# urbste/MultiCol-SLAM

Hardware: AMD Instinct MI355X
Metric: Mfeatures/s extract+match, 3-cam 754x480 multi-frame (higher is better)
Workload: dtype u8+i32 (images, Hamming) / f64 (omni model)

## Files before the change

multicol-slam_amd/csrc/mcs_blur.hip:

```cpp
#include "mcs_common.h"
#include <type_traits>

namespace mcs {

constexpr int kBlurRows = 32;
constexpr int kBlurAhead = 4;

struct BlurLevel { int waveBase, wavesX, rows, ncg; };
struct BlurPlan { int nlevels, totalWaves; BlurLevel lv[MCS_MAX_LEVELS]; };

__device__ __forceinline__ int reflect101(int p, int len) {
	p = p < 0 ? -p : p;
	return p >= len ? 2 * (len - 1) - p : p;
}

__global__ __launch_bounds__(256) void k_blur(ExtractBuffers b, BlurPlan plan, int nimg) {
	const PyrDesc& d = *b.desc;
	const int blk = (blockIdx.x & (kNumXCD - 1)) * (gridDim.x / kNumXCD) + (blockIdx.x / kNumXCD);
	const int wave = __builtin_amdgcn_readfirstlane(blk * 4 + (threadIdx.x >> 6));
	if (wave >= plan.totalWaves) return;
	int level = 0;
	while (level + 1 < plan.nlevels && wave >= plan.lv[level + 1].waveBase) ++level;
	const BlurLevel pl = plan.lv[level];
	const LevelInfo& L = d.lv[level];
	const int w = L.w, h = L.h, dstride = L.stride, pyrBytes = d.pyrBytes;
	const int wl = wave - pl.waveBase;
	const int rb = wl / pl.wavesX, wx = wl - rb * pl.wavesX;
	const int y0 = rb * pl.rows;
	const int nrows = min(pl.rows, h - y0);
	const int items = nimg * pl.ncg;
	const int item0 = wx * 64;
	const int itemRaw = item0 + (threadIdx.x & 63);
	const bool live = itemRaw < items;
	const int item = live ? itemRaw : items - 1;
	const int img = item / pl.ncg, cg = item - img * pl.ncg;
	const int img0 = item0 / pl.ncg;
	const int x = cg * 4;
	int sstride;
	const uint8_t* src = level_ptr(b, d, img0, level, &sstride);
	const size_t simg = level == 0 ? b.img0Pitch : (size_t)pyrBytes;
	uint8_t* dst = b.blur + (size_t)img0 * pyrBytes + L.off;
	const int A = min(max(x - 2, 0), w - 8);
	uint32_t selLo = 0, selHi = 0;
#pragma unroll
	for (int j = 0; j < 8; ++j) {
		const int p = reflect101(min(x - 2 + j, w + 1), w);
// ... 1 lines not shown
		if (j < 4) selLo |= s << (8 * j); else selHi |= s << (8 * (j - 4));
	}
	uint32_t voffS = (uint32_t)((size_t)(img - img0) * simg) + (uint32_t)A;
	uint32_t voffD = (uint32_t)((size_t)(img - img0) * (size_t)pyrBytes) + (uint32_t)x;
	auto loadRow = [&](int it) -> uint2 {
		const int r = reflect101(y0 - 2 + it, h);
		asm volatile("" : "+v"(voffS));
		uint2 v;
		__builtin_memcpy(&v, src + (size_t)((unsigned)r * (unsigned)sstride) + voffS, 8);
		return v;
	};
	const int total = nrows + 4;
	uint2 buf[5];
#pragma unroll
	for (int k = 0; k < kBlurAhead; ++k) buf[k] = loadRow(min(k, total - 1));
	uint32_t ring[5][4];
	uint32_t V[4] = {12u, 12u, 12u, 12u};
	auto body = [&](int it, auto kc, auto firstc, auto storec) {
		constexpr int k = decltype(kc)::value;
		buf[(k + kBlurAhead) % 5] = loadRow(min(it + kBlurAhead, total - 1));
		const uint2 raw = buf[k];
		const uint32_t W0 = __builtin_amdgcn_perm(raw.y, raw.x, selLo), W1 = __builtin_amdgcn_perm(raw.y, raw.x, selHi);
		uint32_t S[4];
		S[0] = __builtin_amdgcn_udot4(W0, 0x01010101u, W1 & 0xffu, false);
		S[1] = __builtin_amdgcn_udot4(W0, 0x01010100u, __builtin_amdgcn_udot4(W1, 0x00000101u, 0u, false), false);
		S[2] = __builtin_amdgcn_udot4(W0, 0x01010000u, __builtin_amdgcn_udot4(W1, 0x00010101u, 0u, false), false);
		S[3] = __builtin_amdgcn_udot4(W0, 0x01000000u, __builtin_amdgcn_udot4(W1, 0x01010101u, 0u, false), false);
#pragma unroll
		for (int c = 0; c < 4; ++c) {
			V[c] += S[c];
			if (!decltype(firstc)::value) V[c] -= ring[k][c];
			ring[k][c] = S[c];
		}
		if (decltype(storec)::value) {
			const uint32_t t0 = __umul24(V[0], 671104u), t1 = __umul24(V[1], 671104u), t2 = __umul24(V[2], 671104u), t3 = __umul24(V[3], 671104u);
			const uint32_t out = __builtin_amdgcn_perm(t1, t0, 0x0c0c0703u) | __builtin_amdgcn_perm(t3, t2, 0x07030c0cu);
			asm volatile("" : "+v"(voffD));
			*reinterpret_cast<uint32_t*>(dst + (size_t)((unsigned)(y0 + it - 4) * (unsigned)dstride) + voffD) = out;
		}
	};
	using T = std::true_type; using F = std::false_type;
	body(0, std::integral_constant<int, 0>(), T(), F()); body(1, std::integral_constant<int, 1>(), T(), F()); body(2, std::integral_constant<int, 2>(), T(), F());
	body(3, std::integral_constant<int, 3>(), T(), F()); body(4, std::integral_constant<int, 4>(), T(), T());
	int it0 = 5;
	for (; it0 + 5 <= total; it0 += 5) {
		body(it0, std::integral_constant<int, 0>(), F(), T()); body(it0 + 1, std::integral_constant<int, 1>(), F(), T()); body(it0 + 2, std::integral_constant<int, 2>(), F(), T());
		body(it0 + 3, std::integral_constant<int, 3>(), F(), T()); body(it0 + 4, std::integral_constant<int, 4>(), F(), T());
	}
	const int rem = total - it0;
	if (rem > 0) body(it0, std::integral_constant<int, 0>(), F(), T());
	if (rem > 1) body(it0 + 1, std::integral_constant<int, 1>(), F(), T());
	if (rem > 2) body(it0 + 2, std::integral_constant<int, 2>(), F(), T());
	if (rem > 3) body(it0 + 3, std::integral_constant<int, 3>(), F(), T());
}

void launch_blur(const ExtractBuffers& b, const PyrDesc& hd, int nimg, hipStream_t s) {
	BlurPlan plan;
	plan.nlevels = hd.nlevels;
	int waves = 0;
	for (int l = 0; l < hd.nlevels; ++l) {
		BlurLevel& p = plan.lv[l];
		const int w = hd.lv[l].w, h = hd.lv[l].h;
		p.ncg = (w + 3) / 4;
		const int nrb = (h + kBlurRows - 1) / kBlurRows;
		p.rows = (h + nrb - 1) / nrb;
		p.wavesX = (nimg * p.ncg + 63) / 64;
		p.waveBase = waves;
		waves += p.wavesX * ((h + p.rows - 1) / p.rows);
	}
	plan.totalWaves = waves;
	hipLaunchKernelGGL(k_blur, dim3(((waves + 3) / 4 + kNumXCD - 1) / kNumXCD * kNumXCD), dim3(256), 0, s, b, plan, nimg);
}

}
```

multicol-slam_amd/csrc/mcs_capi.hip:

```cpp
#include "mcs_extractor.h"
#include "mcs_plan.h"

#include <cstdio>
#include <cstdlib>

namespace mcs {
bool upload_describe_tables(const signed char* pattern);
const signed char kPattern[2048] = {
#include "learned_pattern_64_orb.inc"
};
}

using namespace mcs;

std::string& mcs_err() { static thread_local std::string e; return e; }

static int extractor_build(mcs_extractor* e, const ExtractPlan& plan) {
	const PyrDesc& hd = e->hd;
	if (!upload_describe_tables(kPattern)) return fail(MCS_ERR_HIP, "pattern tables: upload failed (or the distinct-point rounds of mcs_describe.hip do not fit this pattern)");
	const size_t B = e->maxBatch;
#define ALLOC(ptr, bytes) do { hipError_t _e = hipMalloc((void**)&(ptr), (bytes)); if (_e != hipSuccess) return fail(MCS_ERR_HIP, std::string("hipMalloc ") + #ptr + ": " + hipGetErrorString(_e)); } while (0)
	ALLOC(e->d_desc, sizeof(PyrDesc));
	ALLOC(e->d_cells, sizeof(CellInfo) * e->cells.size());
	ALLOC(e->d_taps, sizeof(ResizeTap) * std::max<size_t>(plan.taps.size(), 1));
// ... 67 lines not shown
	else { HIPCHK(hipStreamCreateWithFlags(&c->stream, hipStreamNonBlocking)); c->ownStream = true; }
	if (getenv("MCS_NO_OVERLAP") == nullptr) {
		HIPCHK(hipStreamCreateWithFlags(&c->side, hipStreamNonBlocking));
		auto masked = [&](hipStream_t* st, const char* var) -> hipError_t {
			const char* m = getenv(var);
			if (!m || !*m) return hipStreamCreateWithFlags(st, hipStreamNonBlocking);
			char* end = nullptr;
			const unsigned long v = strtoul(m, &end, 16);
			if (end == m || *end != '\0' || v == 0 || v > 0xFFFFFFFFul) { fprintf(stderr, "mcs: %s=\"%s\" is not a non-zero 32-bit hex word\n", var, m); return hipErrorInvalidValue; }
			uint32_t words[16];
			for (auto& w : words) w = (uint32_t)v;
			hipDeviceProp_t prop;
			if (hipGetDeviceProperties(&prop, device) != hipSuccess) return hipErrorInvalidValue;
			return hipExtStreamCreateWithCUMask(st, (uint32_t)((prop.multiProcessorCount + 31) / 32), words);
		};
		HIPCHK(masked(&c->side2, "MCS_MATCH_CU_MASK"));
		HIPCHK(masked(&c->side3, "MCS_GREEDY_CU_MASK"));
		HIPCHK(hipEventCreateWithFlags(&c->evLists, hipEventDisableTiming));
		for (int i = 0; i < 2; ++i) HIPCHK(hipEventCreateWithFlags(&c->evGreedyBuf[i], hipEventDisableTiming));

		HIPCHK(hipEventCreateWithFlags(&c->evFork, hipEventDisableTiming));
		HIPCHK(hipEventCreateWithFlags(&c->evPyr, hipEventDisableTiming));
		HIPCHK(hipEventCreateWithFlags(&c->evBlur, hipEventDisableTiming));
		HIPCHK(hipEventCreateWithFlags(&c->evMatch, hipEventDisableTiming));
		HIPCHK(hipEventCreateWithFlags(&c->evGreedy, hipEventDisableTiming));
		HIPCHK(hipEventCreateWithFlags(&c->evDescFork, hipEventDisableTiming));
		HIPCHK(hipEventCreateWithFlags(&c->evDescJoin, hipEventDisableTiming));

		for (int i = 0; i < 4; ++i) HIPCHK(hipEventCreateWithFlags(&c->evSearch[i], hipEventDisableTiming));
	}
	*out = c;
	return MCS_OK;
}

int mcs_ctx_join(mcs_ctx* c) {
	if (!c) return fail(MCS_ERR_INVALID, "null ctx");
	return ctx_join_greedy(c, c->stream);
}

int mcs_ctx_set_async_search(mcs_ctx* c, int on) {
	if (!c) return fail(MCS_ERR_INVALID, "null ctx");
	HIPCHK(hipStreamSynchronize(c->stream));
	if (c->side2) { HIPCHK(hipStreamSynchronize(c->side2)); HIPCHK(hipStreamSynchronize(c->side3)); }
	const bool was = c->asyncSearch;
	c->asyncSearch = on != 0 && c->side2 != nullptr;
	if (was != c->asyncSearch) { c->upload = nullptr; c->lastResultStream = nullptr; }
// ... 2 lines not shown

int mcs_ctx_search_fence(mcs_ctx* c, int lag) {
	if (!c || lag < 0 || lag > 2) return fail(MCS_ERR_INVALID, "lag must be 0, 1 or 2");
	if (!c->asyncSearch) return lag == 0 ? mcs_ctx_join(c) : MCS_OK;
	const long long want = c->searchSeq - 1 - lag;
	if (want >= 0) HIPCHK(hipStreamWaitEvent(c->stream, c->evSearch[want & 3], 0));
	if (lag == 0) c->greedyPending = false;
	return MCS_OK;
}

int mcs_ctx_destroy(mcs_ctx* c) {
	if (!c) return MCS_OK;
	(void)hipSetDevice(c->device);
	(void)hipStreamSynchronize(c->stream);
	while (!c->extractors.empty()) (void)mcs_extractor_destroy(c->extractors.back());
	for (auto& kv : c->timers) { if (kv.second.a) { (void)hipEventDestroy(kv.second.a); (void)hipEventDestroy(kv.second.b); } }
	if (c->side) {
		(void)hipStreamSynchronize(c->side);
		(void)hipStreamSynchronize(c->side2);
		(void)hipStreamDestroy(c->side2);
		(void)hipStreamSynchronize(c->side3); (void)hipStreamDestroy(c->side3);
		(void)hipEventDestroy(c->evLists); (void)hipEventDestroy(c->evGreedyBuf[0]); (void)hipEventDestroy(c->evGreedyBuf[1]);
		for (int i = 0; i < 4; ++i) if (c->evSearch[i]) (void)hipEventDestroy(c->evSearch[i]);
		(void)hipEventDestroy(c->evFork); (void)hipEventDestroy(c->evPyr); (void)hipEventDestroy(c->evBlur); (void)hipEventDestroy(c->evMatch); (void)hipEventDestroy(c->evGreedy);
		(void)hipEventDestroy(c->evDescFork); (void)hipEventDestroy(c->evDescJoin);
		(void)hipStreamDestroy(c->side);
	}
	for (hipStream_t ps : c->probed) { (void)hipStreamSynchronize(ps); (void)hipStreamDestroy(ps); }
	if (c->ownStream) (void)hipStreamDestroy(c->stream);
	delete c;
	return MCS_OK;
}

int mcs_ctx_synchronize(mcs_ctx* c) {
	if (!c) return fail(MCS_ERR_INVALID, "null ctx");
	HIPCHK(hipStreamSynchronize(c->stream));
	if (c->side) { HIPCHK(hipStreamSynchronize(c->side)); HIPCHK(hipStreamSynchronize(c->side2)); HIPCHK(hipStreamSynchronize(c->side3)); c->greedyPending = false; }
	return MCS_OK;
}

int mcs_ctx_enable_timing(mcs_ctx* c, int on) {
	if (!c) return fail(MCS_ERR_INVALID, "null ctx");
	if (c->timing != (on != 0)) c->lastResultStream = nullptr;
	c->timing = on != 0;
	return MCS_OK;
}

// ... 74 lines not shown
```

multicol-slam_amd/csrc/mcs_common.h:

```cpp
#pragma once
#include <hip/hip_runtime.h>
#include <vector>
#include <stdint.h>
#include "../../include/mcs_c.h"

namespace mcs {

constexpr int kEdge = 25;
constexpr int kHalfPatch = 16;
constexpr int kPatchSize = 32;
constexpr int kMinBorder = kEdge - 3;
constexpr int kCellW = 30;
constexpr int kMaxRoots = 32;
constexpr int kMaxNodes = 2048;
constexpr int kNumXCD = 8;

struct LevelInfo {
	int w, h, stride;
	int off;
	int nCols, nRows, wCell, hCell;
	int cellBase;
	int capc;
	int slotBase;
	int denseBase, denseCap;
// ... 99 lines not shown
	int* tieCount; uint32_t* tieList;
	unsigned long long* tieTotal;
	double tieBand;
	hipStream_t sideStream; hipEvent_t evDescFork, evDescJoin;
	hipEvent_t evFastA, evFastB;
	double guardEps;
	int describeMode;
	int* nkp; mcs_keypoint* kps; uint8_t* out_desc; uint8_t* out_mask; double* rays;
	size_t outImgPitch; int outRowStride;
};

struct HostLevel { const uint8_t* blur; const uint8_t* raw; int w, h; const uint8_t* patch = nullptr; int prow = 0, pcol = 0, pdim = 0; bool* miss = nullptr; };
constexpr int kTiePatchR = 40;
constexpr int kTiePatchDim = 2 * kTiePatchR + 1;
struct TieCaptureHeader { int count; int status; int pad[14]; };
struct TieCaptureEntry { uint32_t gw; int level; uint32_t rec; float angle; uint8_t patch[kTiePatchDim * kTiePatchDim + 15]; };

__host__ __device__ inline const uint8_t* level_ptr(const ExtractBuffers& b, const PyrDesc& d, int img, int level, int* stride) {
	if (level == 0) { *stride = b.img0Stride; return b.img0 + (size_t)img * b.img0Pitch; }
	*stride = d.lv[level].stride;
	return b.pyr + (size_t)img * d.pyrBytes + d.lv[level].off;
}

void launch_pyramid(const ExtractBuffers& b, const PyrDesc& hd, int nimg, hipStream_t s, int level0 = 1, int level1 = MCS_MAX_LEVELS);
bool pyramid_chain_table(const PyrDesc& d, const ResizeTap* taps, std::vector<int>* table);
void launch_fast(const ExtractBuffers& b, const PyrDesc& hd, int nimg, hipStream_t s, int level0 = 0, int level1 = MCS_MAX_LEVELS);
void launch_octree(const ExtractBuffers& b, const PyrDesc& hd, int nimg, hipStream_t s, int level0 = 0, int level1 = MCS_MAX_LEVELS);
void launch_blur(const ExtractBuffers& b, const PyrDesc& hd, int nimg, hipStream_t s);
void launch_describe(const ExtractBuffers& b, const PyrDesc& hd, int nimg, hipStream_t s);
size_t describe_aux_bytes();

struct RowMap {
	size_t base; int blk; size_t bpitch;
	__device__ __forceinline__ size_t operator()(int i) const {
		if (blk == 0) return base + (size_t)i;
		const int b = i / blk;
		return base + (size_t)b * bpitch + (size_t)(i - b * blk);
	}
};

struct MatchArgs {
	const uint8_t* qd; const uint8_t* qm; const uint8_t* qvalid; const int* qgroup; int nq; int qstride; size_t qpitch;
	const uint8_t* td; const uint8_t* tm; const uint8_t* tvalid; const int* tgroup; int nt; int tstride; size_t tpitch;
	int nsets; int dim; int K; int countThresh;
	int qblk, tblk; size_t qbpitch, tbpitch;
	int toff, tmod;
	int qmod, tdiv;
	int maxDist;
	int splits;
	uint32_t* partial;
	int* partialCount;
// ... 100 lines not shown
```

multicol-slam_amd/csrc/mcs_extract.hip:

```cpp
#include "mcs_extractor.h"
#include "mcs_tiecap.h"

#include <cstdlib>

namespace mcs {
void launch_selftest_fast_model(const OcamDev* cam, const double* tab, unsigned long long seed, int n, int width, int height, unsigned long long* maxDiff, hipStream_t s);

struct ExtractOut { int32_t* nkp; uint32_t* kps; uint32_t* desc; uint32_t* mask; uint32_t* rays; int* status; };
extern "C"
__global__ __launch_bounds__(256) void k_extract_out(const int* __restrict__ d_nkp, const uint32_t* __restrict__ kps, const uint32_t* __restrict__ desc, const uint32_t* __restrict__ mask,
                                                     const uint32_t* __restrict__ rays, const int* __restrict__ d_status, const int* __restrict__ d_ties, ExtractOut o, int kpCap, int descDw,
                                                     ExtractBuffers b, int nimg, int wavesPerImage, int maxTies, uint8_t* __restrict__ tieOut) {
	if ((int)blockIdx.y == nimg) {
		tie_capture_body(b, nimg, wavesPerImage, maxTies, tieOut, blockIdx.x, gridDim.x);
		return;
	}
	const int img = blockIdx.y, n = d_nkp[img], part = blockIdx.x, parts = gridDim.x;
	auto copy = [&](uint32_t* dst, const uint32_t* src, int rowDw) {
		const size_t base = (size_t)img * kpCap * rowDw;
		const int total = n * rowDw;
		for (int i = part * 256 + threadIdx.x; i < total; i += parts * 256) dst[base + i] = src[base + i];
	};
	copy(o.kps, kps, (int)(sizeof(mcs_keypoint) / 4));
	copy(o.desc, desc, descDw);
// ... 126 lines not shown
		HIPCHK(hipMemcpy(e->d_gTab, tabs.data(), tabs.size() * sizeof(double), hipMemcpyHostToDevice));
		e->h_cams = hc;
	}
	if (e->camCache.size() > 64) e->camCache.clear();
	b.cams = e->d_cams;
	return MCS_OK;
}

static void enqueue_describe(mcs_ctx* c, const ExtractBuffers& b, const PyrDesc& hd, int nimg) {
	ExtractBuffers bd = b;
	if (c->timing) {
		Timer& t = c->timers["describe_fast"];
		if (!t.a) { (void)hipEventCreate(&t.a); (void)hipEventCreate(&t.b); }
		bd.evFastA = t.a; bd.evFastB = t.b; t.used = true;
	}
	c->tic("describe"); launch_describe(bd, hd, nimg, c->stream); c->toc("describe");
}

static int enqueue_forked(mcs_ctx* c, ExtractBuffers& b, const PyrDesc& hd, int nimg) {
	hipStream_t s = c->stream;
	HIPCHK(hipEventRecord(c->evFork, s));
	HIPCHK(hipStreamWaitEvent(c->side, c->evFork, 0));
	if (hd.chainFits) {
		launch_pyramid(b, hd, nimg, c->side);
		HIPCHK(hipEventRecord(c->evPyr, c->side));
		launch_blur(b, hd, nimg, c->side);
		HIPCHK(hipEventRecord(c->evBlur, c->side));
		launch_fast(b, hd, nimg, s, 0, 1);
		HIPCHK(hipStreamWaitEvent(s, c->evPyr, 0));
		launch_fast(b, hd, nimg, s, 1, hd.nlevels);
	} else {
		launch_pyramid(b, hd, nimg, c->side, 1, hd.nlevels);
		HIPCHK(hipEventRecord(c->evPyr, c->side));
		launch_blur(b, hd, nimg, c->side);
		HIPCHK(hipEventRecord(c->evBlur, c->side));
		HIPCHK(hipStreamWaitEvent(s, c->evPyr, 0));
		launch_fast(b, hd, nimg, s, 0, hd.nlevels);
	}
	launch_octree(b, hd, nimg, s);
	HIPCHK(hipStreamWaitEvent(s, c->evBlur, 0));
	b.sideStream = c->side; b.evDescFork = c->evDescFork; b.evDescJoin = c->evDescJoin;
	enqueue_describe(c, b, hd, nimg);
	return MCS_OK;
}

static void enqueue_in_order(const ExtractBuffers& b, const PyrDesc& hd, int nimg, hipStream_t s) {
	launch_pyramid(b, hd, nimg, s);
	launch_fast(b, hd, nimg, s);
	launch_octree(b, hd, nimg, s);
	launch_blur(b, hd, nimg, s);
	launch_describe(b, hd, nimg, s);
}

static void graph_evict(mcs_extractor* e, hipStream_t s) {
	if (e->graphs.size() >= 4) { (void)hipStreamSynchronize(s); (void)hipGraphExecDestroy(e->graphs.front().exec); e->graphs.erase(e->graphs.begin()); }
}

static hipGraphExec_t graph_find_or_capture(mcs_extractor* e, const ExtractBuffers& b, int nimg, hipStream_t s) {
	for (mcs_extractor::Graph& g : e->graphs)
		if (g.nimg == nimg && memcmp(&g.key, &b, sizeof(b)) == 0) { ++e->graphHits; return g.exec; }
	++e->graphMisses;
	hipGraphExec_t exec = nullptr;
	hipGraph_t graph = nullptr;
	hipError_t ge = hipStreamBeginCapture(s, hipStreamCaptureModeRelaxed);
	if (ge == hipSuccess) {
		enqueue_in_order(b, e->hd, nimg, s);
		const hipError_t le = hipGetLastError();
		ge = hipStreamEndCapture(s, &graph);
		if (ge == hipSuccess && le != hipSuccess) ge = le;
		if (ge == hipSuccess) ge = hipGraphInstantiate(&exec, graph, nullptr, nullptr, 0);
		if (graph) (void)hipGraphDestroy(graph);
	}
	if (ge != hipSuccess) {
		(void)hipGetLastError();
		e->graphMisses = 1000000;
		return nullptr;
	}
	graph_evict(e, s);
	e->graphs.push_back(mcs_extractor::Graph{b, nimg, exec});
	return exec;
}

static int enqueue_graph(mcs_extractor* e, const ExtractBuffers& b, int nimg) {
	hipStream_t s = e->ctx->stream;
	hipGraphExec_t exec = graph_find_or_capture(e, b, nimg, s);
	if (!exec) enqueue_in_order(b, e->hd, nimg, s);
	else HIPCHK(hipGraphLaunch(exec, s));
	return MCS_OK;
}

static void enqueue_timed(mcs_ctx* c, const ExtractBuffers& b, const PyrDesc& hd, int nimg) {
	hipStream_t s = c->stream;
	c->tic("pyramid"); launch_pyramid(b, hd, nimg, s); c->toc("pyramid");
	c->tic("fast"); launch_fast(b, hd, nimg, s); c->toc("fast");
	c->tic("octree"); launch_octree(b, hd, nimg, s); c->toc("octree");
	c->tic("blur"); launch_blur(b, hd, nimg, s); c->toc("blur");
	enqueue_describe(c, b, hd, nimg);
}

static int finish_host_tail(mcs_extractor* e, hipStream_t s, const int* st, const int* nties, uint8_t* desc, uint8_t* descmask) {
	HIPCHK(hipStreamSynchronize(s));
	if (int r = consume_status(e, *st)) return r;
	if (*nties > 0) { if (int r = fix_ties_host(e, *nties, desc, descmask)) return r; }
	return MCS_OK;
}

static int finish_host(mcs_extractor* e, const ExtractCall& a, const ExtractBuffers& b) {
	const PyrDesc& hd = e->hd;
	hipStream_t s = e->ctx->stream;
	const size_t rows = (size_t)a.nimg * hd.kpCap;
	int st = 0, nties = 0;
	mcs::ExtractOut o{(int32_t*)device_view(a.nkp), (uint32_t*)device_view(a.keypoints), (uint32_t*)device_view(a.desc), (uint32_t*)device_view(a.descmask),
	                  (uint32_t*)device_view(a.rays), e->h_status ? (int*)device_view(e->h_status) : nullptr};
	static const bool outKernel = !(getenv("MCS_OUT_KERNEL") && atoi(getenv("MCS_OUT_KERNEL")) == 0);
	if (outKernel && o.nkp && o.kps && o.desc && o.mask && o.status && (o.rays || !a.rays)) {
		hipLaunchKernelGGL(mcs::k_extract_out, dim3(4, a.nimg + (e->hostTie.dev ? 1 : 0)), dim3(256), 0, s, e->d_nkp, (const uint32_t*)e->d_kps, (const uint32_t*)e->d_odesc, (const uint32_t*)e->d_omask,
		                   (const uint32_t*)e->d_rays, e->d_status, e->d_fbCount + 2, o, hd.kpCap, hd.descSize / 4, b, a.nimg, kp_slots_per_image(hd),
		                   kHostTieSlots, e->hostTie.dev);
		HIPCHK(hipGetLastError());
// ... 149 lines not shown
```

multicol-slam_amd/csrc/mcs_host.h:

```cpp
#pragma once
#include "mcs_common.h"
#include "mcs_carve.h"
#include <algorithm>
#include <cmath>
#include <cstring>
#include <map>
#include <string>
#include <vector>

std::string& mcs_err();
inline int fail(int code, const std::string& msg) { mcs_err() = msg; return code; }
#define HIPCHK(expr)                                                                                       \
	do {                                                                                                   \
		hipError_t _e = (expr);                                                                            \
		if (_e != hipSuccess) return fail(MCS_ERR_HIP, std::string(#expr) + ": " + hipGetErrorString(_e)); \
	} while (0)

static inline int cvRound_(double v) { return (int)lrint(v); }
static inline int cvRoundf_(float v) { return (int)lrintf(v); }
static inline int cvFloor_(double v) { int i = (int)v; return i - (i > v); }
static inline short sat_short(float v) { int iv = cvRoundf_(v); return (short)(iv < -32768 ? -32768 : iv > 32767 ? 32767 : iv); }

struct Timer { hipEvent_t a = nullptr, b = nullptr; bool used = false; };

// ... 40 lines not shown
struct mcs_ctx {
	int device = 0;
	std::vector<mcs_extractor*> extractors;
	hipStream_t stream = nullptr;
	bool ownStream = false;
	bool timing = false;
	std::map<std::string, Timer> timers;
	DevBuf partial, partialCount;
	DevBuf topKeys;
	DevBuf topKeys2;
	DevBuf topCnt;
	DevBuf exA, exW, exRows;
	DevBuf block;
	uint8_t* mirror = nullptr; size_t mirrorCap = 0;
	bool staging = false;
	DevBuf npBuf;
	DevBuf lmBuf;
	void* lbaRec = nullptr;
	hipStream_t side = nullptr;
	hipStream_t side3 = nullptr;
	hipEvent_t evLists = nullptr, evGreedyBuf[2] = {nullptr, nullptr};
	hipStream_t upload = nullptr; unsigned uploadMask = 0; std::vector<hipStream_t> probed; std::vector<unsigned> probedMask;
	hipStream_t side2 = nullptr;
	hipEvent_t evFork = nullptr, evPyr = nullptr, evBlur = nullptr, evMatch = nullptr, evGreedy = nullptr;
	hipEvent_t evDescFork = nullptr, evDescJoin = nullptr;
	bool greedyPending = false;
	bool asyncSearch = false;
	hipEvent_t evSearch[4] = {nullptr, nullptr, nullptr, nullptr};
	long long searchSeq = 0;
	hipStream_t lastResultStream = nullptr;
	bool overlap() const { return side != nullptr && !timing; }

	void tic(const char* name) {
		if (!timing) return;
		Timer& t = timers[name];
		if (!t.a) { (void)hipEventCreate(&t.a); (void)hipEventCreate(&t.b); }
		(void)hipEventRecord(t.a, stream);
	}
	void toc(const char* name) {
		if (!timing) return;
		Timer& t = timers[name];
		(void)hipEventRecord(t.b, stream);
		t.used = true;
	}
	~mcs_ctx() { if (mirror) (void)hipHostFree(mirror); if (lbaRec) (void)hipHostFree(lbaRec); }
};

// ... 81 lines not shown
```

multicol-slam_amd/csrc/mcs_pyramid.hip:

```cpp
#include "mcs_common.h"
#include <type_traits>

namespace mcs {

constexpr int PT_W = 128, PT_H = 32;
constexpr int PS_PITCH = 192;
constexpr int PS_ROWS = 50;

__device__ __forceinline__ uint32_t load_u32_unaligned(const uint8_t* p) {
	uint32_t v;
	__builtin_memcpy(&v, p, 4);
	return v;
}

__attribute__((amdgpu_waves_per_eu(8, 8)))
__global__ __launch_bounds__(256) void k_resize_level(ExtractBuffers b, int level, int tilesX, int tilesY) {
	__shared__ __attribute__((aligned(16))) uint8_t src_t[PS_ROWS * PS_PITCH];
	const PyrDesc& d = *b.desc;
	const LevelInfo& L = d.lv[level];
	const LevelInfo& P = d.lv[level - 1];
	const int img = blockIdx.x / (tilesX * tilesY);
	const int t = blockIdx.x - img * (tilesX * tilesY);
	const int ty = t / tilesX, tx = t - ty * tilesX;
	const int x0 = tx * PT_W, y0 = ty * PT_H;
// ... 79 lines not shown
			const uint8_t* r1 = &src_t[(sy1 - sya) * PS_PITCH];
			emit(y, tyv, [&](int i, int& p00, int& p01, int& p10, int& p11) {
				p00 = r0[col[i]]; p01 = r0[col1[i]]; p10 = r1[col[i]]; p11 = r1[col1[i]];
			});
		}
	} else {
#pragma unroll 1
		for (int j = 0; j < PT_H / 8; ++j) {
			const int y = y0 + (tid >> 5) + 8 * j;
			if (y >= L.h) break;
			const ResizeTap tyv = tapY[y];
			const int sy0 = min(max((int)tyv.ofs, 0), P.h - 1), sy1 = min(max((int)tyv.ofs + 1, 0), P.h - 1);
			const uint8_t* r0 = src + (size_t)sy0 * sstride;
			const uint8_t* r1 = src + (size_t)sy1 * sstride;
			emit(y, tyv, [&](int i, int& p00, int& p01, int& p10, int& p11) {
				const int sx = txv[i].ofs, sx1 = sx + 1 < P.w ? sx + 1 : P.w - 1;
				p00 = r0[sx]; p01 = r0[sx1]; p10 = r1[sx]; p11 = r1[sx1];
			});
		}
	}
}

constexpr int kColsAhead = 3;

__global__ __launch_bounds__(256) void k_resize_cols(ExtractBuffers b, int level, int wavesX, int rows, int ncg, int nimg, int totalWaves) {
	const PyrDesc& d = *b.desc;
	const LevelInfo& L = d.lv[level];
	const LevelInfo& P = d.lv[level - 1];
	const int w = L.w, h = L.h, sw = P.w, sh = P.h, dstride = L.stride, pyrBytes = d.pyrBytes, loff = L.off;
	const ResizeTap* tapX = b.taps + L.tabX;
	const ResizeTap* tapY = b.taps + L.tabY;
	const int blk = (blockIdx.x & (kNumXCD - 1)) * (gridDim.x / kNumXCD) + (blockIdx.x / kNumXCD);
	const int wave = __builtin_amdgcn_readfirstlane(blk * 4 + (threadIdx.x >> 6));
	if (wave >= totalWaves) return;
	const int rb = wave / wavesX, wx = wave - rb * wavesX;
	const int y0 = rb * rows;
	const int nrows = min(rows, h - y0);
	const int lane = threadIdx.x & 63;
	const int items = nimg * ncg;
	const int item0 = wx * 64;
	const int item = min(item0 + lane, items - 1);
	const int img = item / ncg, cg = item - img * ncg;
	const int img0 = item0 / ncg;
	const int x = cg * 4;
	int sstride;
	const uint8_t* src = level_ptr(b, d, img0, level - 1, &sstride);
	const size_t simg = level == 1 ? b.img0Pitch : (size_t)pyrBytes;
	uint8_t* dst = b.pyr + (size_t)img0 * pyrBytes + loff;
	ResizeTap tx[4];
#pragma unroll
	for (int i = 0; i < 4; ++i) tx[i] = tapX[min(x + i, w - 1)];
	const int A = min((int)tx[0].ofs, sw - 8);
	uint32_t sel[4], wt[4], liveMask = 0;
#pragma unroll
	for (int i = 0; i < 4; ++i) {
		const uint32_t c0 = (uint32_t)(tx[i].ofs - A) & 7u, c1 = (uint32_t)(min(tx[i].ofs + 1, sw - 1) - A) & 7u;
		sel[i] = c0 | 0x0c00u | (c1 << 16) | 0x0c000000u;
		wt[i] = (uint32_t)(unsigned short)tx[i].a0 | ((uint32_t)(unsigned short)tx[i].a1 << 16);
		liveMask |= (x + i < w) ? 0xffu << (8 * i) : 0u;
	}
	uint32_t voffS = (uint32_t)((size_t)(img - img0) * simg) + (uint32_t)A;
	uint32_t voffD = (uint32_t)((size_t)(img - img0) * (size_t)pyrBytes) + (uint32_t)x;
	uint32_t tyA, tyB;
	{
		const uint2 t = *reinterpret_cast<const uint2*>(&tapY[min(y0 + lane, h - 1)]);
		tyA = t.x; tyB = t.y;
	}
	auto clipRow = [&](int r) { return min(max(r, 0), sh - 1); };
	const int rs = clipRow((int)(short)(__builtin_amdgcn_readlane(tyA, 0) & 0xffff));
	const int re = clipRow((int)(short)(__builtin_amdgcn_readlane(tyA, nrows - 1) & 0xffff) + 1);
	auto loadRow = [&](int r) -> uint2 {
		asm volatile("" : "+v"(voffS));
		uint2 v;
		__builtin_memcpy(&v, src + (size_t)((unsigned)min(r, re) * (unsigned)sstride) + voffS, 8);
		return v;
	};
	uint2 raw[4];
#pragma unroll
	for (int k = 0; k < kColsAhead; ++k) raw[k] = loadRow(rs + k);
	uint32_t T[2][4];
#pragma unroll
	for (int i = 0; i < 4; ++i) T[0][i] = T[1][i] = 0;
	int yi = 0;
	int sy = (int)(short)(__builtin_amdgcn_readlane(tyA, 0) & 0xffff);
	auto emit = [&](const uint32_t* T0, const uint32_t* T1) {
		const uint32_t b0 = __builtin_amdgcn_readlane(tyA, yi) & 0xffff0000u;
		const uint32_t b1 = __builtin_amdgcn_readlane(tyB, yi) << 16;
		uint32_t v[4];
#pragma unroll
		for (int i = 0; i < 4; ++i) v[i] = (__umulhi(T0[i], b0) + __umulhi(T1[i], b1) + 2u) >> 2;
		const uint32_t out = (v[0] | (v[1] << 8) | (v[2] << 16) | (v[3] << 24)) & liveMask;
		asm volatile("" : "+v"(voffD));
		*reinterpret_cast<uint32_t*>(dst + (size_t)((unsigned)(y0 + yi) * (unsigned)dstride) + voffD) = out;
	};
	auto body = [&](int r, auto kc) {
		constexpr int K = decltype(kc)::value;
		raw[(K + kColsAhead) % 4] = loadRow(r + kColsAhead);
		uint32_t* cur = T[K & 1];
		const uint32_t* prev = T[(K & 1) ^ 1];
		typedef unsigned short us2 __attribute__((ext_vector_type(2)));
#pragma unroll
		for (int i = 0; i < 4; ++i)
			cur[i] = __builtin_amdgcn_udot2(__builtin_bit_cast(us2, __builtin_amdgcn_perm(raw[K].y, raw[K].x, sel[i])), __builtin_bit_cast(us2, wt[i]), 0u, false) >> 4;
		while (yi < nrows && clipRow(sy + 1) == r) {
			if (clipRow(sy) == r) emit(cur, cur);
			else emit(prev, cur);
			++yi;
			sy = (int)(short)(__builtin_amdgcn_readlane(tyA, min(yi, nrows - 1)) & 0xffff);
		}
	};
	int r = rs;
	for (; r + 3 <= re; r += 4) {
		body(r, std::integral_constant<int, 0>()); body(r + 1, std::integral_constant<int, 1>());
		body(r + 2, std::integral_constant<int, 2>()); body(r + 3, std::integral_constant<int, 3>());
	}
	if (r <= re) body(r, std::integral_constant<int, 0>());
	if (r + 1 <= re) body(r + 1, std::integral_constant<int, 1>());
	if (r + 2 <= re) body(r + 2, std::integral_constant<int, 2>());
}

constexpr int FT_W = 64, FT_H = 16;
constexpr int FA_PITCH = 288, FA_ROWS = 72;
constexpr int FB_PITCH = 232, FB_ROWS = 60;
constexpr int FUSED_MAX_W = 256;
constexpr int kChainLevels = 8;

struct ChainRegion { int xa, xb, ya, yb; int oxs, oxe, oys, oye; };

static void chain_regions(const PyrDesc& d, const ResizeTap* taps, int top, int tx, int ty, int tilesX, int tilesY, ChainRegion* R) {
	const LevelInfo& T = d.lv[top];
	ChainRegion r;
	r.xa = tx * FT_W; r.xb = (tx == tilesX - 1 ? T.w : r.xa + FT_W) - 1;
	r.ya = ty * FT_H; r.yb = (ty == tilesY - 1 ? T.h : r.ya + FT_H) - 1;
	r.oxs = r.xa; r.oxe = tx == tilesX - 1 ? (T.w + 3) & ~3 : r.xa + FT_W;
	r.oys = r.ya; r.oye = r.yb + 1;
	R[top] = r;
	for (int l = top; l >= 1; --l) {
		const LevelInfo& L = d.lv[l];
		const LevelInfo& P = d.lv[l - 1];
		const ResizeTap* tapX = taps + L.tabX;
		const ResizeTap* tapY = taps + L.tabY;
// ... 122 lines not shown
				const int sy0 = min(max((int)tyv.ofs, 0), P.h - 1), sy1 = min(max((int)tyv.ofs + 1, 0), P.h - 1);
				const uint8_t* r0 = &sbuf[(sy0 - sr.ya) * sp];
				const uint8_t* r1 = &sbuf[(sy1 - sr.ya) * sp];
				int p00[4], p01[4], p10[4], p11[4];
#pragma unroll
				for (int i = 0; i < 4; ++i) { p00[i] = r0[col[i]]; p01[i] = r0[col1[i]]; p10[i] = r1[col[i]]; p11[i] = r1[col1[i]]; }
				uint32_t packed = 0;
#pragma unroll
				for (int i = 0; i < 4; ++i) {
					const int t0 = p00[i] * txv[i].a0 + p01[i] * txv[i].a1;
					const int t1 = p10[i] * txv[i].a0 + p11[i] * txv[i].a1;
					const int v = ((((int)tyv.a0 * (t0 >> 4)) >> 16) + (((int)tyv.a1 * (t1 >> 4)) >> 16) + 2) >> 2;
					packed |= (uint32_t)(v & 0xff) << (8 * i);
				}
				packed &= live;
				if (l < top) *reinterpret_cast<uint32_t*>(&dbuf[(y - c.ya) * dp + 4 * cg]) = packed;
				if (ownX && y >= c.oys && y < c.oye) *reinterpret_cast<uint32_t*>(dst + (unsigned)y * (unsigned)L.stride + (unsigned)x4) = packed;
			}
		}
		__syncthreads();
	}
}

void launch_pyramid(const ExtractBuffers& b, const PyrDesc& hd, int nimg, hipStream_t s, int level0, int level1) {
	if (level0 <= 1 && level1 >= hd.nlevels && hd.chainFits && hd.nlevels > 1) {
		const int top = hd.nlevels - 1;
		const int tilesX = (hd.lv[top].w + FT_W - 1) / FT_W, tilesY = (hd.lv[top].h + FT_H - 1) / FT_H;
		hipLaunchKernelGGL(k_resize_chain, dim3(nimg * tilesX * tilesY), dim3(256), 0, s, b, tilesX, tilesY);
		return;
	}
	static const bool tileOnly = getenv("MCS_PYR_TILES") != nullptr;
	for (int level = level0 < 1 ? 1 : level0; level < hd.nlevels && level < level1; ++level) {
		const LevelInfo& L = hd.lv[level];
		if (L.colsOk && !tileOnly) {
			const int ncg = (L.w + 3) / 4, wavesX = (nimg * ncg + 63) / 64;
			int nrb = (L.h + 31) / 32;
			while (wavesX * nrb < 4096 && (L.h + nrb - 1) / nrb > 8) ++nrb;
			const int rows = (L.h + nrb - 1) / nrb;
			const int waves = wavesX * ((L.h + rows - 1) / rows);
			hipLaunchKernelGGL(k_resize_cols, dim3(((waves + 3) / 4 + kNumXCD - 1) / kNumXCD * kNumXCD), dim3(256), 0, s, b, level, wavesX, rows, ncg, nimg, waves);
			continue;
		}
		const int tilesX = (L.w + PT_W - 1) / PT_W, tilesY = (L.h + PT_H - 1) / PT_H;
		hipLaunchKernelGGL(k_resize_level, dim3(nimg * tilesX * tilesY), dim3(256), 0, s, b, level, tilesX, tilesY);
	}
}

}
```

Before: 148.9.

## Fuse 5x5 box blur into column-resize pyramid kernel for resized levels

Adds a templated blur variant of the column resize kernel that computes each resized row, exchanges neighbouring pixels across lanes with DPP, and produces the 5x5 box blur in registers through a row ring. This writes blurred output directly, so those levels skip the separate blur pass and no longer reload the pyramid from memory. The blur kernel now takes a level mask and handles only the levels not already blurred. The cost is overlapping halo rows and columns per wave (62 owned items per wave, two extra rows on each side), which means redundant resize work. An optional env setting also forks the level-0 blur onto a separate stream.

```diff
diff --git a/multicol-slam_amd/csrc/mcs_blur.hip b/multicol-slam_amd/csrc/mcs_blur.hip
--- a/multicol-slam_amd/csrc/mcs_blur.hip
+++ b/multicol-slam_amd/csrc/mcs_blur.hip
@@ -1,4 +1,5 @@
 #include "mcs_common.h"
+#include "mcs_box5.h"
 #include <type_traits>
 
 namespace mcs {
@@ -6,22 +7,18 @@
 constexpr int kBlurRows = 32;
 constexpr int kBlurAhead = 4;
 
-struct BlurLevel { int waveBase, wavesX, rows, ncg; };
+struct BlurLevel { int level, waveBase, wavesX, rows, ncg; };
 struct BlurPlan { int nlevels, totalWaves; BlurLevel lv[MCS_MAX_LEVELS]; };
-
-__device__ __forceinline__ int reflect101(int p, int len) {
-	p = p < 0 ? -p : p;
-	return p >= len ? 2 * (len - 1) - p : p;
-}
 
 __global__ __launch_bounds__(256) void k_blur(ExtractBuffers b, BlurPlan plan, int nimg) {
 	const PyrDesc& d = *b.desc;
 	const int blk = (blockIdx.x & (kNumXCD - 1)) * (gridDim.x / kNumXCD) + (blockIdx.x / kNumXCD);
 	const int wave = __builtin_amdgcn_readfirstlane(blk * 4 + (threadIdx.x >> 6));
 	if (wave >= plan.totalWaves) return;
-	int level = 0;
-	while (level + 1 < plan.nlevels && wave >= plan.lv[level + 1].waveBase) ++level;
-	const BlurLevel pl = plan.lv[level];
+	int entry = 0;
+	while (entry + 1 < plan.nlevels && wave >= plan.lv[entry + 1].waveBase) ++entry;
+	const BlurLevel pl = plan.lv[entry];
+	const int level = pl.level;
 	const LevelInfo& L = d.lv[level];
 	const int w = L.w, h = L.h, dstride = L.stride, pyrBytes = d.pyrBytes;
 	const int wl = wave - pl.waveBase;
@@ -69,10 +66,7 @@
 		const uint2 raw = buf[k];
 		const uint32_t W0 = __builtin_amdgcn_perm(raw.y, raw.x, selLo), W1 = __builtin_amdgcn_perm(raw.y, raw.x, selHi);
 		uint32_t S[4];
-		S[0] = __builtin_amdgcn_udot4(W0, 0x01010101u, W1 & 0xffu, false);
-		S[1] = __builtin_amdgcn_udot4(W0, 0x01010100u, __builtin_amdgcn_udot4(W1, 0x00000101u, 0u, false), false);
-		S[2] = __builtin_amdgcn_udot4(W0, 0x01010000u, __builtin_amdgcn_udot4(W1, 0x00010101u, 0u, false), false);
-		S[3] = __builtin_amdgcn_udot4(W0, 0x01000000u, __builtin_amdgcn_udot4(W1, 0x01010101u, 0u, false), false);
+		box5_hsums(W0, W1, S);
 #pragma unroll
 		for (int c = 0; c < 4; ++c) {
 			V[c] += S[c];
@@ -80,8 +74,7 @@
 			ring[k][c] = S[c];
 		}
 		if (decltype(storec)::value) {
-			const uint32_t t0 = __umul24(V[0], 671104u), t1 = __umul24(V[1], 671104u), t2 = __umul24(V[2], 671104u), t3 = __umul24(V[3], 671104u);
-			const uint32_t out = __builtin_amdgcn_perm(t1, t0, 0x0c0c0703u) | __builtin_amdgcn_perm(t3, t2, 0x07030c0cu);
+			const uint32_t out = box5_div25(V[0], V[1], V[2], V[3]);
 			asm volatile("" : "+v"(voffD));
 			*reinterpret_cast<uint32_t*>(dst + (size_t)((unsigned)(y0 + it - 4) * (unsigned)dstride) + voffD) = out;
 		}
@@ -101,12 +94,14 @@
 	if (rem > 3) body(it0 + 3, std::integral_constant<int, 3>(), F(), T());
 }
 
-void launch_blur(const ExtractBuffers& b, const PyrDesc& hd, int nimg, hipStream_t s) {
+void launch_blur(const ExtractBuffers& b, const PyrDesc& hd, int nimg, hipStream_t s, unsigned levels) {
 	BlurPlan plan;
-	plan.nlevels = hd.nlevels;
+	plan.nlevels = 0;
 	int waves = 0;
 	for (int l = 0; l < hd.nlevels; ++l) {
-		BlurLevel& p = plan.lv[l];
+		if (!(levels >> l & 1u)) continue;
+		BlurLevel& p = plan.lv[plan.nlevels++];
+		p.level = l;
 		const int w = hd.lv[l].w, h = hd.lv[l].h;
 		p.ncg = (w + 3) / 4;
 		const int nrb = (h + kBlurRows - 1) / kBlurRows;
@@ -116,6 +111,7 @@
 		waves += p.wavesX * ((h + p.rows - 1) / p.rows);
 	}
 	plan.totalWaves = waves;
+	if (waves == 0) return;
 	hipLaunchKernelGGL(k_blur, dim3(((waves + 3) / 4 + kNumXCD - 1) / kNumXCD * kNumXCD), dim3(256), 0, s, b, plan, nimg);
 }
 
diff --git a/multicol-slam_amd/csrc/mcs_box5.h b/multicol-slam_amd/csrc/mcs_box5.h
--- /dev/null
+++ b/multicol-slam_amd/csrc/mcs_box5.h
@@ -0,0 +1,24 @@
+#pragma once
+#include <stdint.h>
+#include <hip/hip_runtime.h>
+
+namespace mcs {
+
+__device__ __forceinline__ int reflect101(int p, int len) {
+	p = p < 0 ? -p : p;
+	return p >= len ? 2 * (len - 1) - p : p;
+}
+
+__device__ __forceinline__ void box5_hsums(uint32_t W0, uint32_t W1, uint32_t S[4]) {
+	S[0] = __builtin_amdgcn_udot4(W0, 0x01010101u, W1 & 0xffu, false);
+	S[1] = __builtin_amdgcn_udot4(W0, 0x01010100u, __builtin_amdgcn_udot4(W1, 0x00000101u, 0u, false), false);
+	S[2] = __builtin_amdgcn_udot4(W0, 0x01010000u, __builtin_amdgcn_udot4(W1, 0x00010101u, 0u, false), false);
+	S[3] = __builtin_amdgcn_udot4(W0, 0x01000000u, __builtin_amdgcn_udot4(W1, 0x01010101u, 0u, false), false);
+}
+
+__device__ __forceinline__ uint32_t box5_div25(uint32_t V0, uint32_t V1, uint32_t V2, uint32_t V3) {
+	const uint32_t t0 = __umul24(V0, 671104u), t1 = __umul24(V1, 671104u), t2 = __umul24(V2, 671104u), t3 = __umul24(V3, 671104u);
+	return __builtin_amdgcn_perm(t1, t0, 0x0c0c0703u) | __builtin_amdgcn_perm(t3, t2, 0x07030c0cu);
+}
+
+}
diff --git a/multicol-slam_amd/csrc/mcs_capi.hip b/multicol-slam_amd/csrc/mcs_capi.hip
--- a/multicol-slam_amd/csrc/mcs_capi.hip
+++ b/multicol-slam_amd/csrc/mcs_capi.hip
@@ -113,6 +113,7 @@
 		HIPCHK(hipEventCreateWithFlags(&c->evFork, hipEventDisableTiming));
 		HIPCHK(hipEventCreateWithFlags(&c->evPyr, hipEventDisableTiming));
 		HIPCHK(hipEventCreateWithFlags(&c->evBlur, hipEventDisableTiming));
+		HIPCHK(hipEventCreateWithFlags(&c->evBlur0, hipEventDisableTiming));
 		HIPCHK(hipEventCreateWithFlags(&c->evMatch, hipEventDisableTiming));
 		HIPCHK(hipEventCreateWithFlags(&c->evGreedy, hipEventDisableTiming));
 		HIPCHK(hipEventCreateWithFlags(&c->evDescFork, hipEventDisableTiming));
@@ -161,7 +162,7 @@
 		(void)hipStreamSynchronize(c->side3); (void)hipStreamDestroy(c->side3);
 		(void)hipEventDestroy(c->evLists); (void)hipEventDestroy(c->evGreedyBuf[0]); (void)hipEventDestroy(c->evGreedyBuf[1]);
 		for (int i = 0; i < 4; ++i) if (c->evSearch[i]) (void)hipEventDestroy(c->evSearch[i]);
-		(void)hipEventDestroy(c->evFork); (void)hipEventDestroy(c->evPyr); (void)hipEventDestroy(c->evBlur); (void)hipEventDestroy(c->evMatch); (void)hipEventDestroy(c->evGreedy);
+		(void)hipEventDestroy(c->evFork); (void)hipEventDestroy(c->evPyr); (void)hipEventDestroy(c->evBlur); (void)hipEventDestroy(c->evBlur0); (void)hipEventDestroy(c->evMatch); (void)hipEventDestroy(c->evGreedy);
 		(void)hipEventDestroy(c->evDescFork); (void)hipEventDestroy(c->evDescJoin);
 		(void)hipStreamDestroy(c->side);
 	}
diff --git a/multicol-slam_amd/csrc/mcs_common.h b/multicol-slam_amd/csrc/mcs_common.h
--- a/multicol-slam_amd/csrc/mcs_common.h
+++ b/multicol-slam_amd/csrc/mcs_common.h
@@ -145,11 +145,12 @@
 	return b.pyr + (size_t)img * d.pyrBytes + d.lv[level].off;
 }
 
-void launch_pyramid(const ExtractBuffers& b, const PyrDesc& hd, int nimg, hipStream_t s, int level0 = 1, int level1 = MCS_MAX_LEVELS);
+unsigned launch_pyramid(const ExtractBuffers& b, const PyrDesc& hd, int nimg, hipStream_t s, int level0 = 1, int level1 = MCS_MAX_LEVELS);
+inline unsigned all_levels(const PyrDesc& hd) { return (1u << hd.nlevels) - 1u; }
 bool pyramid_chain_table(const PyrDesc& d, const ResizeTap* taps, std::vector<int>* table);
 void launch_fast(const ExtractBuffers& b, const PyrDesc& hd, int nimg, hipStream_t s, int level0 = 0, int level1 = MCS_MAX_LEVELS);
 void launch_octree(const ExtractBuffers& b, const PyrDesc& hd, int nimg, hipStream_t s, int level0 = 0, int level1 = MCS_MAX_LEVELS);
-void launch_blur(const ExtractBuffers& b, const PyrDesc& hd, int nimg, hipStream_t s);
+void launch_blur(const ExtractBuffers& b, const PyrDesc& hd, int nimg, hipStream_t s, unsigned levels);
 void launch_describe(const ExtractBuffers& b, const PyrDesc& hd, int nimg, hipStream_t s);
 size_t describe_aux_bytes();
 
diff --git a/multicol-slam_amd/csrc/mcs_extract.hip b/multicol-slam_amd/csrc/mcs_extract.hip
--- a/multicol-slam_amd/csrc/mcs_extract.hip
+++ b/multicol-slam_amd/csrc/mcs_extract.hip
@@ -172,17 +172,26 @@
 	HIPCHK(hipEventRecord(c->evFork, s));
 	HIPCHK(hipStreamWaitEvent(c->side, c->evFork, 0));
 	if (hd.chainFits) {
-		launch_pyramid(b, hd, nimg, c->side);
+		const unsigned blurred = launch_pyramid(b, hd, nimg, c->side);
 		HIPCHK(hipEventRecord(c->evPyr, c->side));
-		launch_blur(b, hd, nimg, c->side);
+		launch_blur(b, hd, nimg, c->side, all_levels(hd) & ~blurred);
 		HIPCHK(hipEventRecord(c->evBlur, c->side));
 		launch_fast(b, hd, nimg, s, 0, 1);
 		HIPCHK(hipStreamWaitEvent(s, c->evPyr, 0));
 		launch_fast(b, hd, nimg, s, 1, hd.nlevels);
 	} else {
-		launch_pyramid(b, hd, nimg, c->side, 1, hd.nlevels);
+		static const bool blur0Fork = getenv("MCS_PYR_BLUR") && atoi(getenv("MCS_PYR_BLUR")) == 2;
+		const unsigned blurred = launch_pyramid(b, hd, nimg, c->side, 1, hd.nlevels);
 		HIPCHK(hipEventRecord(c->evPyr, c->side));
-		launch_blur(b, hd, nimg, c->side);
+		unsigned rest = all_levels(hd) & ~blurred;
+		if (blur0Fork && blurred) {
+			HIPCHK(hipStreamWaitEvent(c->side3, c->evFork, 0));
+			launch_blur(b, hd, nimg, c->side3, 1u);
+			HIPCHK(hipEventRecord(c->evBlur0, c->side3));
+			HIPCHK(hipStreamWaitEvent(c->side, c->evBlur0, 0));
+			rest &= ~1u;
+		}
+		launch_blur(b, hd, nimg, c->side, rest);
 		HIPCHK(hipEventRecord(c->evBlur, c->side));
 		HIPCHK(hipStreamWaitEvent(s, c->evPyr, 0));
 		launch_fast(b, hd, nimg, s, 0, hd.nlevels);
@@ -195,10 +204,10 @@
 }
 
 static void enqueue_in_order(const ExtractBuffers& b, const PyrDesc& hd, int nimg, hipStream_t s) {
-	launch_pyramid(b, hd, nimg, s);
+	const unsigned blurred = launch_pyramid(b, hd, nimg, s);
 	launch_fast(b, hd, nimg, s);
 	launch_octree(b, hd, nimg, s);
-	launch_blur(b, hd, nimg, s);
+	launch_blur(b, hd, nimg, s, all_levels(hd) & ~blurred);
 	launch_describe(b, hd, nimg, s);
 }
 
@@ -241,10 +250,10 @@
 
 static void enqueue_timed(mcs_ctx* c, const ExtractBuffers& b, const PyrDesc& hd, int nimg) {
 	hipStream_t s = c->stream;
-	c->tic("pyramid"); launch_pyramid(b, hd, nimg, s); c->toc("pyramid");
+	c->tic("pyramid"); const unsigned blurred = launch_pyramid(b, hd, nimg, s); c->toc("pyramid");
 	c->tic("fast"); launch_fast(b, hd, nimg, s); c->toc("fast");
 	c->tic("octree"); launch_octree(b, hd, nimg, s); c->toc("octree");
-	c->tic("blur"); launch_blur(b, hd, nimg, s); c->toc("blur");
+	c->tic("blur"); launch_blur(b, hd, nimg, s, all_levels(hd) & ~blurred); c->toc("blur");
 	enqueue_describe(c, b, hd, nimg);
 }
 
diff --git a/multicol-slam_amd/csrc/mcs_host.h b/multicol-slam_amd/csrc/mcs_host.h
--- a/multicol-slam_amd/csrc/mcs_host.h
+++ b/multicol-slam_amd/csrc/mcs_host.h
@@ -86,7 +86,7 @@
 	hipEvent_t evLists = nullptr, evGreedyBuf[2] = {nullptr, nullptr};
 	hipStream_t upload = nullptr; unsigned uploadMask = 0; std::vector<hipStream_t> probed; std::vector<unsigned> probedMask;
 	hipStream_t side2 = nullptr;
-	hipEvent_t evFork = nullptr, evPyr = nullptr, evBlur = nullptr, evMatch = nullptr, evGreedy = nullptr;
+	hipEvent_t evFork = nullptr, evPyr = nullptr, evBlur = nullptr, evBlur0 = nullptr, evMatch = nullptr, evGreedy = nullptr;
 	hipEvent_t evDescFork = nullptr, evDescJoin = nullptr;
 	bool greedyPending = false;
 	bool asyncSearch = false;
diff --git a/multicol-slam_amd/csrc/mcs_pyramid.hip b/multicol-slam_amd/csrc/mcs_pyramid.hip
--- a/multicol-slam_amd/csrc/mcs_pyramid.hip
+++ b/multicol-slam_amd/csrc/mcs_pyramid.hip
@@ -1,4 +1,5 @@
 #include "mcs_common.h"
+#include "mcs_box5.h"
 #include <type_traits>
 
 namespace mcs {
@@ -125,7 +126,10 @@
 }
 
 constexpr int kColsAhead = 3;
-
+constexpr int kFusedItems = 62;
+constexpr int kFusedMaxRows = 60;
+
+template <bool BLUR>
 __global__ __launch_bounds__(256) void k_resize_cols(ExtractBuffers b, int level, int wavesX, int rows, int ncg, int nimg, int totalWaves) {
 	const PyrDesc& d = *b.desc;
 	const LevelInfo& L = d.lv[level];
@@ -137,12 +141,15 @@
 	const int wave = __builtin_amdgcn_readfirstlane(blk * 4 + (threadIdx.x >> 6));
 	if (wave >= totalWaves) return;
 	const int rb = wave / wavesX, wx = wave - rb * wavesX;
-	const int y0 = rb * rows;
-	const int nrows = min(rows, h - y0);
+	const int y0 = BLUR ? max(rb * rows - 2, 0) : rb * rows;
+	const int nrows = BLUR ? min(rb * rows + rows + 2, h) - y0 : min(rows, h - y0);
+	const int own0 = rb * rows, own1 = min(own0 + rows, h);
 	const int lane = threadIdx.x & 63;
 	const int items = nimg * ncg;
-	const int item0 = wx * 64;
-	const int item = min(item0 + lane, items - 1);
+	const int item0 = BLUR ? max(wx * kFusedItems - 1, 0) : wx * 64;
+	const int itemRaw = (BLUR ? wx * kFusedItems - 1 : wx * 64) + lane;
+	const int item = BLUR ? min(max(itemRaw, 0), items - 1) : min(itemRaw, items - 1);
+	const bool owner = !BLUR || (lane >= 1 && lane <= kFusedItems && itemRaw < items);
 	const int img = item / ncg, cg = item - img * ncg;
 	const int img0 = item0 / ncg;
 	const int x = cg * 4;
@@ -164,6 +171,35 @@
 	}
 	uint32_t voffS = (uint32_t)((size_t)(img - img0) * simg) + (uint32_t)A;
 	uint32_t voffD = (uint32_t)((size_t)(img - img0) * (size_t)pyrBytes) + (uint32_t)x;
+	uint32_t bselLo = 0, bselHi = 0;
+	const bool lastCg = cg == ncg - 1;
+	uint8_t* bdst = nullptr;
+	if constexpr (BLUR) {
+#pragma unroll
+		for (int j = 0; j < 8; ++j) {
+			const int p = reflect101(min(x - 2 + j, w + 1), w);
+			if (j < 4) bselLo |= ((uint32_t)(p - (x - 4)) & 7u) << (8 * j);
+			else bselHi |= ((uint32_t)(p - x) & 7u) << (8 * (j - 4));
+		}
+		bdst = b.blur + (size_t)img0 * pyrBytes + loff;
+	}
+	uint32_t ringS[4][2];
+#pragma unroll
+	for (int k = 0; k < 4; ++k) ringS[k][0] = ringS[k][1] = 0;
+	auto blurPush = [&](uint32_t s01, uint32_t s23, int ye) {
+		if (own0 == 0 && ye == 2) { ringS[2][0] = ringS[0][0]; ringS[2][1] = ringS[0][1]; ringS[3][0] = s01; ringS[3][1] = s23; }
+		const int yo = ye - 2;
+		if (yo >= own0 && yo < own1) {
+			const uint32_t v01 = s01 + ringS[0][0] + ringS[1][0] + ringS[2][0] + ringS[3][0] + 0x000c000cu;
+			const uint32_t v23 = s23 + ringS[0][1] + ringS[1][1] + ringS[2][1] + ringS[3][1] + 0x000c000cu;
+			const uint32_t out = box5_div25(v01 & 0xffffu, v01 >> 16, v23 & 0xffffu, v23 >> 16);
+			asm volatile("" : "+v"(voffD));
+			if (owner) *reinterpret_cast<uint32_t*>(bdst + (size_t)((unsigned)yo * (unsigned)dstride) + voffD) = out;
+		}
+#pragma unroll
+		for (int k = 3; k > 0; --k) { ringS[k][0] = ringS[k - 1][0]; ringS[k][1] = ringS[k - 1][1]; }
+		ringS[0][0] = s01; ringS[0][1] = s23;
+	};
 	uint32_t tyA, tyB;
 	{
 		const uint2 t = *reinterpret_cast<const uint2*>(&tapY[min(y0 + lane, h - 1)]);
@@ -192,9 +228,24 @@
 		uint32_t v[4];
 #pragma unroll
 		for (int i = 0; i < 4; ++i) v[i] = (__umulhi(T0[i], b0) + __umulhi(T1[i], b1) + 2u) >> 2;
-		const uint32_t out = (v[0] | (v[1] << 8) | (v[2] << 16) | (v[3] << 24)) & liveMask;
-		asm volatile("" : "+v"(voffD));
-		*reinterpret_cast<uint32_t*>(dst + (size_t)((unsigned)(y0 + yi) * (unsigned)dstride) + voffD) = out;
+		if constexpr (!BLUR) {
+			const uint32_t out = (v[0] | (v[1] << 8) | (v[2] << 16) | (v[3] << 24)) & liveMask;
+			asm volatile("" : "+v"(voffD));
+			*reinterpret_cast<uint32_t*>(dst + (size_t)((unsigned)(y0 + yi) * (unsigned)dstride) + voffD) = out;
+		} else {
+			const uint32_t pix = v[0] | (v[1] << 8) | (v[2] << 16) | (v[3] << 24);
+			const int y = y0 + yi;
+			if (y >= own0 && y < own1) {
+				asm volatile("" : "+v"(voffD));
+				if (owner) *reinterpret_cast<uint32_t*>(dst + (size_t)((unsigned)y * (unsigned)dstride) + voffD) = pix & liveMask;
+			}
+			const uint32_t left = (uint32_t)__builtin_amdgcn_update_dpp((int)pix, (int)pix, 0x138, 0xf, 0xf, false);
+			const uint32_t right = (uint32_t)__builtin_amdgcn_update_dpp((int)pix, (int)pix, 0x130, 0xf, 0xf, false);
+			const uint32_t W0 = __builtin_amdgcn_perm(pix, left, bselLo), W1 = __builtin_amdgcn_perm(lastCg ? left : right, pix, bselHi);
+			uint32_t S[4];
+			box5_hsums(W0, W1, S);
+			blurPush(S[0] | (S[1] << 16), S[2] | (S[3] << 16), y);
+		}
 	};
 	auto body = [&](int r, auto kc) {
 		constexpr int K = decltype(kc)::value;
@@ -220,6 +271,12 @@
 	if (r <= re) body(r, std::integral_constant<int, 0>());
 	if (r + 1 <= re) body(r + 1, std::integral_constant<int, 1>());
 	if (r + 2 <= re) body(r + 2, std::integral_constant<int, 2>());
+	if constexpr (BLUR) {
+		if (y0 + nrows == h) {
+			blurPush(ringS[1][0], ringS[1][1], h);
+			blurPush(ringS[3][0], ringS[3][1], h + 1);
+		}
+	}
 }
 
 constexpr int FT_W = 64, FT_H = 16;
@@ -388,28 +445,48 @@
 	}
 }
 
-void launch_pyramid(const ExtractBuffers& b, const PyrDesc& hd, int nimg, hipStream_t s, int level0, int level1) {
+constexpr int kFusedMinRows = 16;
+static int fused_rows(int h, int wavesX) {
+	int nrb = (h + 31) / 32;
+	while (wavesX * nrb < 4096 && (h + nrb - 1) / nrb > kFusedMinRows) ++nrb;
+	return (h + nrb - 1) / nrb;
+}
+static_assert(kFusedMinRows >= 4 && 32 <= kFusedMaxRows, "a block below the first starts at row own0 - 2 >= 2; own rows + 4 halo rows fit the wave's 64 row taps");
+
+unsigned launch_pyramid(const ExtractBuffers& b, const PyrDesc& hd, int nimg, hipStream_t s, int level0, int level1) {
 	if (level0 <= 1 && level1 >= hd.nlevels && hd.chainFits && hd.nlevels > 1) {
 		const int top = hd.nlevels - 1;
 		const int tilesX = (hd.lv[top].w + FT_W - 1) / FT_W, tilesY = (hd.lv[top].h + FT_H - 1) / FT_H;
 		hipLaunchKernelGGL(k_resize_chain, dim3(nimg * tilesX * tilesY), dim3(256), 0, s, b, tilesX, tilesY);
-		return;
+		return 0u;
 	}
 	static const bool tileOnly = getenv("MCS_PYR_TILES") != nullptr;
+	static const bool fuseBlur = !(getenv("MCS_PYR_BLUR") && atoi(getenv("MCS_PYR_BLUR")) == 0);
+	unsigned blurred = 0;
 	for (int level = level0 < 1 ? 1 : level0; level < hd.nlevels && level < level1; ++level) {
 		const LevelInfo& L = hd.lv[level];
 		if (L.colsOk && !tileOnly) {
-			const int ncg = (L.w + 3) / 4, wavesX = (nimg * ncg + 63) / 64;
+			const int ncg = (L.w + 3) / 4;
+			if (fuseBlur && L.w >= 8 && L.h >= 5) {
+				const int wavesX = (nimg * ncg + kFusedItems - 1) / kFusedItems;
+				const int rows = fused_rows(L.h, wavesX);
+				const int waves = wavesX * ((L.h + rows - 1) / rows);
+				hipLaunchKernelGGL(k_resize_cols<true>, dim3(((waves + 3) / 4 + kNumXCD - 1) / kNumXCD * kNumXCD), dim3(256), 0, s, b, level, wavesX, rows, ncg, nimg, waves);
+				blurred |= 1u << level;
+				continue;
+			}
+			const int wavesX = (nimg * ncg + 63) / 64;
 			int nrb = (L.h + 31) / 32;
 			while (wavesX * nrb < 4096 && (L.h + nrb - 1) / nrb > 8) ++nrb;
 			const int rows = (L.h + nrb - 1) / nrb;
 			const int waves = wavesX * ((L.h + rows - 1) / rows);
-			hipLaunchKernelGGL(k_resize_cols, dim3(((waves + 3) / 4 + kNumXCD - 1) / kNumXCD * kNumXCD), dim3(256), 0, s, b, level, wavesX, rows, ncg, nimg, waves);
+			hipLaunchKernelGGL(k_resize_cols<false>, dim3(((waves + 3) / 4 + kNumXCD - 1) / kNumXCD * kNumXCD), dim3(256), 0, s, b, level, wavesX, rows, ncg, nimg, waves);
 			continue;
 		}
 		const int tilesX = (L.w + PT_W - 1) / PT_W, tilesY = (L.h + PT_H - 1) / PT_H;
 		hipLaunchKernelGGL(k_resize_level, dim3(nimg * tilesX * tilesY), dim3(256), 0, s, b, level, tilesX, tilesY);
 	}
-}
-
-}
+	return blurred;
+}
+
+}
```

Result: slower. 143.1 (-3.9%).
